# cmavro/GNN-RAG

Hardware: NVIDIA H100
Metric: questions/sec (GNN forward+score) on WebQSP-shape subgraphs; agg-kernel HBM GB/s (higher is better)
Workload: dtype f32

## Files before the change

gnn_rag_b200/csrc/linear_tc.cu:

```cuda
#include "wgmma.cuh"

namespace gr {

int g_tc_cluster = 1;
int g_tc_bk = 32;
int g_tc_tma_store = 1;

namespace {

using namespace tc;
constexpr int kThreads = 384;
constexpr int kConsumerWarps = 8;
constexpr int kLaunchRegs = 168, kProducerRegs = 40, kConsumerRegs = 232;
static_assert(128 * kProducerRegs + 256 * kConsumerRegs <= kThreads * kLaunchRegs, "register budget");

__global__ void split_bf16_seg_kernel(const float* __restrict__ W, int64_t ldw, int64_t N, int64_t Kpad,
                                      int seg, int pitch, __nv_bfloat16* __restrict__ hi,
                                      __nv_bfloat16* __restrict__ lo, int64_t ldo) {
  const int64_t total = N * Kpad;
  const int64_t stride = (int64_t)gridDim.x * blockDim.x;
  for (int64_t i = (int64_t)blockIdx.x * blockDim.x + threadIdx.x; i < total; i += stride) {
    const int64_t n = i / Kpad, k = i - n * Kpad;
    const int sidx = (int)(k / pitch), c = (int)(k - (int64_t)sidx * pitch);
    float v = c < seg ? __ldg(W + n * ldw + (int64_t)sidx * seg + c) : 0.f;
    const __nv_bfloat16 h = __float2bfloat16_rn(v);
    hi[n * ldo + k] = h;
    lo[n * ldo + k] = __float2bfloat16_rn(v - __bfloat162float(h));
  }
}

__global__ void split_bf16_kernel(const float* __restrict__ A, int64_t lda, int64_t M, int64_t K,
                                  __nv_bfloat16* __restrict__ hi, __nv_bfloat16* __restrict__ lo,
                                  int64_t ldo, int vec_ok, int vec_st) {
  const int64_t kq = (K + 3) / 4;
  const int64_t total = M * kq;
  const int64_t stride = (int64_t)gridDim.x * blockDim.x;
  for (int64_t i = (int64_t)blockIdx.x * blockDim.x + threadIdx.x; i < total; i += stride) {
// ... 19 lines not shown
    if (vec_st && k + 3 < ldo) {
      *reinterpret_cast<uint2*>(ph) = *reinterpret_cast<uint2*>(h);
      *reinterpret_cast<uint2*>(pl) = *reinterpret_cast<uint2*>(l);
    } else {
#pragma unroll
      for (int q = 0; q < 4; ++q)
        if (k + q < ldo) { ph[q] = h[q]; pl[q] = l[q]; }
    }
  }
}

struct TcParams {
  const float* bias;
  float* C;
  int64_t ldc;
  __nv_bfloat16* c_hi;
  __nv_bfloat16* c_lo;
  int64_t ldc16;
  const float* w_score;
  float* dots;
  int M, N, K, n_pad, n16, stages, num_tiles;
  uint32_t flags;
  int tma_store;
  int kg_T, kg_G, kg_pitch, kg_nkb, kg_one0, kg_one1, kg_nb0;
};

template <int NP, int CS, int BK, bool GROUPED>
__global__ void __launch_bounds__(kThreads, 1)
linear_tc_kernel(const __grid_constant__ CUtensorMap map_a_hi, const __grid_constant__ CUtensorMap map_a_lo,
                 const __grid_constant__ CUtensorMap map_w_hi, const __grid_constant__ CUtensorMap map_w_lo,
                 const __grid_constant__ CUtensorMap map_c, const __grid_constant__ CUtensorMap map_c_hi,
                 const __grid_constant__ CUtensorMap map_c_lo, const TcParams p) {
  extern __shared__ __align__(1024) uint8_t smem_raw[];
  uint8_t* smem = reinterpret_cast<uint8_t*>((reinterpret_cast<uintptr_t>(smem_raw) + 1023) & ~(uintptr_t)1023);
  const int a_bytes = BM * BK * 2;
  constexpr int w_bytes = NP * BK * 2;
  const bool single = (p.flags & GR_LINEAR_BF16_SINGLE) != 0;
  const int w_off = single ? a_bytes : 2 * a_bytes;
  const int stage_bytes = single ? a_bytes + w_bytes : 2 * a_bytes + 2 * w_bytes;
  uint8_t* s_out = smem + (size_t)p.stages * stage_bytes;
  uint64_t* bars = reinterpret_cast<uint64_t*>(s_out + 2 * kStageOutBytes);
  uint64_t* full_bar = bars;
  uint64_t* empty_bar = bars + p.stages;
  float* s_bias = reinterpret_cast<float*>(bars + 2 * p.stages);
  float* s_ws = s_bias + 256;
  for (int i = threadIdx.x; i < 256; i += kThreads) {
    s_bias[i] = (p.bias && i < p.N) ? p.bias[i] : 0.f;
    s_ws[i] = (p.w_score && i < p.N) ? p.w_score[i] : 0.f;
  }

  const int warp = threadIdx.x >> 5, lane = threadIdx.x & 31;
  const int nkb = GROUPED ? p.kg_nkb : (p.K + BK - 1) / BK;
  const int crank = CS > 1 ? (int)cluster_ctarank() : 0;
  const int ncluster = gridDim.x / CS, cid = blockIdx.x / CS;
  const int ngroups = (p.num_tiles + CS - 1) / CS;
  constexpr uint16_t kMask = (uint16_t)((1u << CS) - 1);

  if (threadIdx.x == 0) {
    for (int s = 0; s < p.stages; ++s) {
      mbar_init(&full_bar[s], 1);
      mbar_init(&empty_bar[s], kConsumerWarps * CS);
    }
    asm volatile("fence.mbarrier_init.release.cluster;" ::: "memory");
  }
  __syncthreads();
  if (CS > 1) cluster_sync_all();

  if (warp < 4) {
    asm volatile("setmaxnreg.dec.sync.aligned.u32 %0;" ::"n"(kProducerRegs));
    if (warp == 0 && lane == 0) {
      uint32_t phase = 0;
      int s = 0;
      constexpr int w_rows = NP / CS;
      const int w_slice = w_rows * BK * 2;
      for (int g = cid; g < ngroups; g += ncluster) {
        const int m0 = (g * CS + crank) * BM;
        for (int kb = 0; kb < nkb; ++kb) {
          mbar_wait(&empty_bar[s], phase ^ 1);
          uint8_t* st = smem + (size_t)s * stage_bytes;
          mbar_expect_tx(&full_bar[s], (uint32_t)stage_bytes);
          int a_col = kb * BK;
          if constexpr (GROUPED) {
            if (p.kg_nb0 == 0) {
              const int g = kb / p.kg_T, t = kb - g * p.kg_T, ni = p.kg_T >> 1;
              const int seg = t == 0 ? 0 : 1 + 2 * ((t - 1) % ni) + (t - 1) / ni;
              a_col = seg * p.kg_pitch + g * BK;
            } else {
              const int g = min(kb / p.kg_T, p.kg_G), t = kb - g * p.kg_T;
              a_col = t == 0 ? g * BK : p.kg_nb0 + (kb - g - 1) * BK;
            }
          }
          tma_load_2d(st, &map_a_hi, &full_bar[s], a_col, m0);
          if (!single) tma_load_2d(st + a_bytes, &map_a_lo, &full_bar[s], a_col, m0);
          if (CS == 1) {
            tma_load_2d(st + w_off, &map_w_hi, &full_bar[s], kb * BK, 0);
            if (!single) tma_load_2d(st + w_off + w_bytes, &map_w_lo, &full_bar[s], kb * BK, 0);
          } else {
            tma_load_2d_mc(st + w_off + crank * w_slice, &map_w_hi, &full_bar[s], kb * BK,
                           crank * w_rows, kMask);
            if (!single)
              tma_load_2d_mc(st + w_off + w_bytes + crank * w_slice, &map_w_lo, &full_bar[s], kb * BK,
                             crank * w_rows, kMask);
          }
          if (++s == p.stages) { s = 0; phase ^= 1; }
        }
      }
    }
  } else {
    asm volatile("setmaxnreg.inc.sync.aligned.u32 %0;" ::"n"(kConsumerRegs));
    const int cw = (warp - 4) >> 2, wq = warp & 3;
    const EpiOut e{s_bias, s_ws, (p.flags & GR_LINEAR_RELU) != 0};
    const int r = wq * 16 + (lane >> 2), cq = lane & 3;
    uint8_t* stg = s_out + (size_t)cw * kStageOutBytes;
    const bool issuer = wq == 0 && lane == 0;
    const bool vec_c = p.C && (p.ldc % 2 == 0) && ((reinterpret_cast<uintptr_t>(p.C) & 7) == 0);
    const bool vec_h = p.c_hi && (p.ldc16 % 2 == 0) && ((reinterpret_cast<uintptr_t>(p.c_hi) & 3) == 0) &&
                       ((reinterpret_cast<uintptr_t>(p.c_lo) & 3) == 0);
    uint32_t phase = 0;
    int s = 0;
    for (int g = cid; g < ngroups; g += ncluster) {
      const int tile = g * CS + crank;
      float acc[NP / 2];
#pragma unroll
      for (int i = 0; i < NP / 2; ++i) acc[i] = 0.f;
      int prev = -1;
      for (int kb = 0; kb < nkb; ++kb) {
        mbar_wait(&full_bar[s], phase);
        const uint32_t sa = smem_u32(smem + (size_t)s * stage_bytes);
        const uint32_t a_row = (uint32_t)(cw * WG_M * BK * 2);
        const uint64_t da_hi = make_smem_desc<BK>(sa + a_row), da_lo = make_smem_desc<BK>(sa + a_bytes + a_row);
        const uint64_t dw_hi = make_smem_desc<BK>(sa + w_off), dw_lo = make_smem_desc<BK>(sa + w_off + w_bytes);
        if constexpr (GROUPED) {
          if (kb >= p.kg_one0 && kb < p.kg_one1) mma_kblock<NP, BK, 1, false>(acc, da_hi, da_lo, dw_hi, dw_lo);
          else mma_kblock<NP, BK, BK / MMA_K, false>(acc, da_hi, da_lo, dw_hi, dw_lo);
        } else if (single) {
          mma_kblock<NP, BK, BK / MMA_K, true>(acc, da_hi, da_lo, dw_hi, dw_lo);
        } else {
          mma_kblock<NP, BK, BK / MMA_K, false>(acc, da_hi, da_lo, dw_hi, dw_lo);
        }
        wgmma_wait<1>();
        if (prev >= 0 && lane == 0) release_slot<CS>(&empty_bar[prev]);
        prev = s;
        if (++s == p.stages) { s = 0; phase ^= 1; }
      }
      wgmma_wait<0>();
      if (prev >= 0 && lane == 0) release_slot<CS>(&empty_bar[prev]);

      const int64_t row0 = (int64_t)tile * BM + cw * WG_M + r;
      float dot0 = 0.f, dot1 = 0.f;
#pragma unroll
      for (int q = 0; q < NP / 16; ++q) {
        const int c0 = 16 * q;
        if (c0 >= p.n_pad) continue;
        float v[8];
        epi_values(acc, q, cq, e, v, dot0, dot1);
        if (p.tma_store) {
          epi_store_tma(v, stg, r, cq, issuer, 1 + cw, &map_c, &map_c_hi, &map_c_lo, p.C != nullptr,
                        p.c_hi != nullptr, c0, tile * BM + cw * WG_M);
          continue;
        }
#pragma unroll
        for (int b = 0; b < 2; ++b) {
          const int col = c0 + 8 * b + 2 * cq;
#pragma unroll
          for (int hr = 0; hr < 2; ++hr) {
            const int64_t row = row0 + 8 * hr;
            if (row >= p.M) continue;
            const float x0 = v[4 * b + 2 * hr], x1 = v[4 * b + 2 * hr + 1];
            if (p.C) {
              float* c = p.C + row * p.ldc + col;
              if (vec_c && col + 1 < p.N) {
                *reinterpret_cast<float2*>(c) = make_float2(x0, x1);
              } else {
                if (col < p.N) c[0] = x0;
                if (col + 1 < p.N) c[1] = x1;
              }
            }
            if (p.c_hi) {
              uint32_t lo;
              const uint32_t hi = split_hi_lo(x0, x1, lo);
              unsigned short* ph = reinterpret_cast<unsigned short*>(p.c_hi + row * p.ldc16 + col);
              unsigned short* pl = reinterpret_cast<unsigned short*>(p.c_lo + row * p.ldc16 + col);
              if (vec_h && col + 1 < p.n16) {
                *reinterpret_cast<uint32_t*>(ph) = hi;
                *reinterpret_cast<uint32_t*>(pl) = lo;
              } else {
                if (col < p.n16) { ph[0] = (unsigned short)(hi & 0xFFFF); pl[0] = (unsigned short)(lo & 0xFFFF); }
                if (col + 1 < p.n16) { ph[1] = (unsigned short)(hi >> 16); pl[1] = (unsigned short)(lo >> 16); }
              }
            }
          }
        }
      }
      epi_dots(dot0, dot1, p.dots, row0, p.M, cq);
    }
    if (p.tma_store && issuer) asm volatile("cp.async.bulk.wait_group 0;" ::: "memory");
  }
  __syncthreads();
  if (CS > 1) cluster_sync_all();
}

struct TcPlan {
  int64_t kp;
  int n_pad, np, stages, bk;
  size_t a_plane_bytes, w_plane_bytes, total_bytes, w_only_bytes, smem_bytes;
  bool ok;
};

TcPlan plan_tc(int64_t M, int64_t N, int64_t K, bool single = false) {
  TcPlan t{};
  const int BK = g_tc_bk == 64 ? 64 : 32;
  t.ok = (N >= 8 && N <= 256 && K >= 8 && M >= 1);
  t.kp = (K + 7) / 8 * 8;
  t.n_pad = (int)((N + 15) / 16 * 16);
  t.np = t.n_pad <= 64 ? 64 : t.n_pad <= 128 ? 128 : t.n_pad <= 208 ? 208 : 256;
  const size_t stage = (single ? 1 : 2) * ((size_t)BM * BK * 2 + (size_t)t.np * BK * 2);
  int stages = (int)((227 * 1024 - 1024 - 2048 - 128 - 2 * kStageOutBytes) / stage);
  t.stages = stages > 8 ? 8 : stages;
  if (t.stages < 2) t.ok = false;
  t.bk = BK;
  t.smem_bytes = (size_t)t.stages * stage + 1024  + 2 * t.stages * 8 + 2 * 256 * 4 + 2 * kStageOutBytes;
  t.a_plane_bytes = align_up((size_t)M * t.kp * 2, 256);
  t.w_plane_bytes = align_up((size_t)N * t.kp * 2, 256);
  t.total_bytes = 2 * t.a_plane_bytes + 2 * t.w_plane_bytes;
  t.w_only_bytes = 2 * t.w_plane_bytes;
  return t;
}


int split_launch(const float* A, int64_t lda, int64_t M, int64_t K, __nv_bfloat16* hi, __nv_bfloat16* lo,
                 int64_t ldo, cudaStream_t stream) {
  int va = (lda % 4 == 0) && ((reinterpret_cast<uintptr_t>(A) & 15) == 0);
  int64_t work = M * ((K + 3) / 4);
  int grid = (int)std::min<int64_t>(ceil_div(work, 256), 32LL * sm_count());
  int vs = (ldo % 4 == 0) && ((reinterpret_cast<uintptr_t>(hi) & 7) == 0) &&
           ((reinterpret_cast<uintptr_t>(lo) & 7) == 0);
  split_bf16_kernel<<<grid, 256, 0, stream>>>(A, lda, M, K, hi, lo, ldo, va, vs);
  GR_CHECK_LAUNCH();
  return GR_OK;
}

template <int NP, int CS, int BK, bool GROUPED = false>
int launch_tc_cs(const CUtensorMap& m_a_hi, const CUtensorMap& m_a_lo, const CUtensorMap& m_w_hi,
                 const CUtensorMap& m_w_lo, const CUtensorMap& m_c, const CUtensorMap& m_c_hi,
                 const CUtensorMap& m_c_lo, const TcPlan& t, const TcParams& p, cudaStream_t stream) {
  const int ngroups = (p.num_tiles + CS - 1) / CS;
  const int nclusters = std::max(1, std::min(ngroups, sm_count() / CS));
  return launch_cluster<linear_tc_kernel<NP, CS, BK, GROUPED>>("gr_linear_tc", kLaunchRegs, CS, nclusters * CS, kThreads,
                                                               t.smem_bytes, stream, m_a_hi, m_a_lo, m_w_hi, m_w_lo,
                                                               m_c, m_c_hi, m_c_lo, p);
}

template <int NP>
int launch_tc_np(const CUtensorMap* const (&m)[7], int cs, const TcPlan& t, const TcParams& p, cudaStream_t stream) {
  if (p.kg_T) {
    if (cs == 2) return launch_tc_cs<NP, 2, 32, true>(*m[0], *m[1], *m[2], *m[3], *m[4], *m[5], *m[6], t, p, stream);
    return launch_tc_cs<NP, 1, 32, true>(*m[0], *m[1], *m[2], *m[3], *m[4], *m[5], *m[6], t, p, stream);
  }
  if (t.bk == 64) {
    if (cs == 2) return launch_tc_cs<NP, 2, 64>(*m[0], *m[1], *m[2], *m[3], *m[4], *m[5], *m[6], t, p, stream);
    return launch_tc_cs<NP, 1, 64>(*m[0], *m[1], *m[2], *m[3], *m[4], *m[5], *m[6], t, p, stream);
  }
  if (cs == 2) return launch_tc_cs<NP, 2, 32>(*m[0], *m[1], *m[2], *m[3], *m[4], *m[5], *m[6], t, p, stream);
  return launch_tc_cs<NP, 1, 32>(*m[0], *m[1], *m[2], *m[3], *m[4], *m[5], *m[6], t, p, stream);
}

int launch_tc(const __nv_bfloat16* a_hi, const __nv_bfloat16* a_lo, int64_t lda16,
              const __nv_bfloat16* w_hi, const __nv_bfloat16* w_lo, int64_t ldw16, const TcPlan& t,
              TcParams p, cudaStream_t stream) {
  p.n_pad = t.n_pad; p.stages = t.stages;
  p.num_tiles = (int)ceil_div(p.M, BM);
  int cs = (g_tc_cluster >= 2 && (t.np / 2) % 8 == 0 && p.num_tiles >= 2) ? 2 : 1;
  CUtensorMap m_a_hi, m_a_lo, m_w_hi, m_w_lo;
  const int64_t w_cols = p.kg_T ? ldw16 : p.K;
  const int64_t a_cols = p.kg_nb0 ? p.kg_nb0 + (int64_t)(p.kg_T - 1) * p.kg_pitch : p.K;
  if (!make_tmap(&m_a_hi, a_hi, p.M, a_cols, lda16, BM, t.bk) || !make_tmap(&m_a_lo, a_lo, p.M, a_cols, lda16, BM, t.bk) ||
      !make_tmap(&m_w_hi, w_hi, p.N, w_cols, ldw16, t.np / cs, t.bk) ||
      !make_tmap(&m_w_lo, w_lo, p.N, w_cols, ldw16, t.np / cs, t.bk)) {
    set_error("gr_linear_tc: cuTensorMapEncodeTiled failed (pointers must be 16-byte aligned, row strides "
              "multiples of 8 elements)");
    return GR_ERR_CUDA;
  }
  p.n16 = (int)std::min<int64_t>((p.N + 15) / 16 * 16, p.ldc16);
  CUtensorMap m_c, m_c_hi, m_c_lo;
  memset(&m_c, 0, sizeof(m_c)); memset(&m_c_hi, 0, sizeof(m_c_hi)); memset(&m_c_lo, 0, sizeof(m_c_lo));
  bool ok = g_tc_tma_store != 0;
  if (ok && p.C) ok = p.N % 4 == 0 && make_out_tmap(&m_c, p.C, p.M, p.N, p.ldc, 4);
  if (ok && p.c_hi) ok = make_out_tmap(&m_c_hi, p.c_hi, p.M, p.n16, p.ldc16, 2) &&
                         make_out_tmap(&m_c_lo, p.c_lo, p.M, p.n16, p.ldc16, 2);
  p.tma_store = ok ? 1 : 0;
  const CUtensorMap* m[7] = {&m_a_hi, &m_a_lo, &m_w_hi, &m_w_lo, &m_c, &m_c_hi, &m_c_lo};
  switch (t.np) {
    case 64: return launch_tc_np<64>(m, cs, t, p, stream);
    case 128: return launch_tc_np<128>(m, cs, t, p, stream);
    case 208: return launch_tc_np<208>(m, cs, t, p, stream);
    default: return launch_tc_np<256>(m, cs, t, p, stream);
  }
}

}

bool linear_tc_supported(int64_t M, int64_t N, int64_t K) {
  return plan_tc(M, N, K).ok && get_encode_fn() != nullptr;
}

}

extern "C" size_t gr_linear_tc_workspace_bytes(int64_t M, int64_t N, int64_t K) {
  if (M <= 0 || N <= 0 || K <= 0) return 0;
  return gr::plan_tc(M, N, K).total_bytes;
}

extern "C" size_t gr_linear_tc_planes_workspace_bytes(int64_t N, int64_t K) {
  if (N <= 0 || K <= 0) return 0;
  return gr::plan_tc(1, N, K).w_only_bytes;
}

extern "C" int gr_split_bf16(const float* A, int64_t lda, int64_t M, int64_t K, void* hi, void* lo,
                             int64_t ld_out, void* stream_) {
  using namespace gr;
  GR_CHECK_ARG(A && hi && lo, "null pointer");
  GR_CHECK_ARG(M > 0 && K > 0 && lda >= K && ld_out >= K && ld_out % 8 == 0, "bad shape / ld_out % 8 != 0");
  return split_launch(A, lda, M, K, reinterpret_cast<__nv_bfloat16*>(hi), reinterpret_cast<__nv_bfloat16*>(lo),
                      ld_out, reinterpret_cast<cudaStream_t>(stream_));
}

extern "C" int gr_linear_tc(const float* A, int64_t lda, const float* W, int64_t ldw, const float* bias,
                            float* C, int64_t ldc, int64_t M, int64_t N, int64_t K, uint32_t flags,
                            void* workspace, size_t workspace_bytes, void* stream_) {
  using namespace gr;
  cudaStream_t stream = reinterpret_cast<cudaStream_t>(stream_);
  GR_CHECK_ARG(A && W && C && workspace, "null pointer");
  GR_CHECK_ARG(M > 0 && N > 0 && K > 0, "M, N, K must be positive");
  GR_CHECK_ARG(lda >= K && ldw >= K && ldc >= N, "leading dimension smaller than row length");
  GR_CHECK_ARG(M < (int64_t)0x7fffffff - BM, "M exceeds int32 range");
  TcPlan t = plan_tc(M, N, K);
  if (!t.ok) {
    set_error("gr_linear_tc: unsupported shape M=%lld N=%lld K=%lld (need 8 <= N <= 256, K >= 8)",
              (long long)M, (long long)N, (long long)K);
    return GR_ERR_UNSUPPORTED;
  }
  if (int rc = check_workspace(__func__, workspace, workspace_bytes, t.total_bytes)) return rc;
  if ((reinterpret_cast<uintptr_t>(workspace) & 255) != 0) {
    set_error("gr_linear_tc: workspace must be 256-byte aligned");
    return GR_ERR_INVALID_ARG;
  }
  char* ws = reinterpret_cast<char*>(workspace);
  __nv_bfloat16* a_hi = reinterpret_cast<__nv_bfloat16*>(ws);
  __nv_bfloat16* a_lo = reinterpret_cast<__nv_bfloat16*>(ws + t.a_plane_bytes);
  __nv_bfloat16* w_hi = reinterpret_cast<__nv_bfloat16*>(ws + 2 * t.a_plane_bytes);
  __nv_bfloat16* w_lo = reinterpret_cast<__nv_bfloat16*>(ws + 2 * t.a_plane_bytes + t.w_plane_bytes);
  int rc = split_launch(A, lda, M, K, a_hi, a_lo, t.kp, stream);
  if (rc != GR_OK) return rc;
  rc = split_launch(W, ldw, N, K, w_hi, w_lo, t.kp, stream);
  if (rc != GR_OK) return rc;
  TcParams p{};
  p.bias = bias; p.C = C; p.ldc = ldc;
  p.M = (int)M; p.N = (int)N; p.K = (int)K; p.flags = flags;
// ... 8 lines not shown
  using namespace gr;
  cudaStream_t stream = reinterpret_cast<cudaStream_t>(stream_);
  GR_CHECK_ARG(A_hi && (A_lo || (flags & GR_LINEAR_BF16_SINGLE)) && W && workspace, "null pointer");
  GR_CHECK_ARG(C || C_hi, "no output requested");
  GR_CHECK_ARG(M > 0 && N > 0 && K > 0, "M, N, K must be positive");
  const bool grouped = (flags & GR_LINEAR_K_GROUPED) != 0;
  const bool korder = (flags & GR_LINEAR_K_ORDER_PLANES) != 0;
  GR_CHECK_ARG(!korder || grouped, "GR_LINEAR_K_ORDER_PLANES modifies GR_LINEAR_K_GROUPED and needs it");
  if (grouped) {
    GR_CHECK_ARG(k_seg > 0 && k_seg_pitch >= k_seg && k_seg_pitch % 16 == 0,
                 "GR_LINEAR_K_GROUPED needs segmented K: k_seg > 0 and k_seg_pitch >= k_seg, a multiple of 16");
    GR_CHECK_ARG(K % k_seg_pitch == 0 && (K / k_seg_pitch) % 2 == 1,
                 "GR_LINEAR_K_GROUPED needs an odd number of segments (2 I + 1)");
    GR_CHECK_ARG(g_tc_bk != 64, "GR_LINEAR_K_GROUPED needs 32-column k-blocks (tc_bk = 32)");
    GR_CHECK_ARG(!(flags & GR_LINEAR_BF16_SINGLE), "GR_LINEAR_K_GROUPED does not combine with GR_LINEAR_BF16_SINGLE");
  }
  const bool segmented = grouped || (k_seg > 0 && k_seg_pitch > k_seg);
  GR_CHECK_ARG(lda16 >= K && lda16 % 8 == 0, "lda16 must be >= K and a multiple of 8");
  GR_CHECK_ARG(!segmented || K % k_seg_pitch == 0, "K must be a multiple of k_seg_pitch");
  GR_CHECK_ARG(ldw >= (segmented ? K / k_seg_pitch * k_seg : K), "ldw smaller than the weight row length");
  GR_CHECK_ARG(!C || ldc >= N, "ldc smaller than N");
  GR_CHECK_ARG(!C_hi || (C_lo && ldc16 >= N), "C_lo missing or ldc16 smaller than N");
  GR_CHECK_ARG(!dots || w_score, "dots requested without w_score");
  GR_CHECK_ARG(M < (int64_t)0x7fffffff - BM, "M exceeds int32 range");
  TcPlan t = plan_tc(M, N, K, (flags & GR_LINEAR_BF16_SINGLE) != 0);
  if (!t.ok) {
    set_error("gr_linear_tc_planes: unsupported shape M=%lld N=%lld K=%lld", (long long)M, (long long)N,
              (long long)K);
    return GR_ERR_UNSUPPORTED;
  }
  const int num_ins = grouped ? (int)(K / k_seg_pitch / 2) : 0;
  const GroupedK gk = grouped ? plan_grouped_k(k_seg_pitch, num_ins, N, korder) : GroupedK{};
  const int64_t nb0 = (k_seg_pitch + 31) / 32 * 32;
  GR_CHECK_ARG(!korder || lda16 >= nb0 + 2 * num_ins * k_seg_pitch,
               "GR_LINEAR_K_ORDER_PLANES: lda16 must cover the neighbour region (round32(k_seg_pitch) + (K - k_seg_pitch) "
               "columns)");
  const size_t w_plane_bytes = grouped ? gk.w_plane_bytes : t.w_plane_bytes;
  if (workspace_bytes < 2 * w_plane_bytes || (reinterpret_cast<uintptr_t>(workspace) & 255) != 0) {
    set_error("gr_linear_tc_planes: workspace too small or not 256-byte aligned");
    return GR_ERR_WORKSPACE;
  }
  char* ws = reinterpret_cast<char*>(workspace);
  __nv_bfloat16* w_hi = reinterpret_cast<__nv_bfloat16*>(ws);
  __nv_bfloat16* w_lo = reinterpret_cast<__nv_bfloat16*>(ws + w_plane_bytes);
  int rc = GR_OK;
  if (flags & GR_LINEAR_W_PRESPLIT) {
  } else if (grouped) {
// ... 31 lines not shown
```

gnn_rag_b200/csrc/wgmma.cuh:

```cuda
#pragma once
#include <cuda.h>
#include <cuda_bf16.h>

#include "common.cuh"

namespace gr {
namespace tc {

constexpr int BM = 128;
constexpr int WG_M = 64;
constexpr int MMA_K = 16;

struct GroupedK {
  int G, ksteps_last, nkb;
  int64_t kp;
  size_t w_plane_bytes;
};
GroupedK plan_grouped_k(int64_t pitch, int I, int64_t N_out, bool packed = false);
int grouped_w_split(const float* W, int64_t ldw, int64_t N_out, int D, int I, const GroupedK& k, __nv_bfloat16* hi,
                    __nv_bfloat16* lo, cudaStream_t stream);

typedef CUresult (*EncodeTiledFn)(CUtensorMap*, CUtensorMapDataType, cuuint32_t, void*, const cuuint64_t*,
                                  const cuuint64_t*, const cuuint32_t*, const cuuint32_t*,
                                  CUtensorMapInterleave, CUtensorMapSwizzle, CUtensorMapL2promotion,
// ... 166 lines not shown
  } else if constexpr (N == 32) {
    GR_WGMMA(32, GR_REGS16, 16, 17, GR_ACC8(0), GR_ACC8(8));
  } else if constexpr (N == 64) {
    GR_WGMMA(64, GR_REGS32, 32, 33, GR_ACC32(0));
  } else if constexpr (N == 128) {
    GR_WGMMA(128, GR_REGS64, 64, 65, GR_ACC32(0), GR_ACC32(32));
  } else if constexpr (N == 208) {
    GR_WGMMA(208, GR_REGS104, 104, 105, GR_ACC32(0), GR_ACC32(32), GR_ACC32(64), GR_ACC8(96));
  } else {
    static_assert(N == 256, "instruction widths: 16, 32, 64, 128, 208, 256");
    GR_WGMMA(256, GR_REGS128, 128, 129, GR_ACC32(0), GR_ACC32(32), GR_ACC32(64), GR_ACC32(96));
  }
}
#undef GR_WGMMA
#undef GR_REGS128
#undef GR_REGS104
#undef GR_REGS64
#undef GR_REGS32
#undef GR_REGS16
#undef GR_REGS8
#undef GR_ACC32
#undef GR_ACC8

template <int NP, int NI, int BK, int C0 = 0>
__device__ __forceinline__ void wgmma_product(float (&acc)[NP / 2], uint64_t a, uint64_t b) {
  constexpr int n = NP - C0 < NI ? NP - C0 : NI;
  wgmma_bf16<n, C0 / 2>(acc, a, b + (uint64_t)((C0 * BK * 2) >> 4));
  if constexpr (C0 + n < NP) wgmma_product<NP, NI, BK, C0 + n>(acc, a, b);
}

template <int NP, int BK, int KSTEPS, bool SINGLE, int NI = NP>
__device__ __forceinline__ void mma_kblock(float (&acc)[NP / 2], uint64_t da_hi, uint64_t da_lo, uint64_t dw_hi,
                                           uint64_t dw_lo) {
  static_assert(KSTEPS >= 1 && KSTEPS <= BK / MMA_K, "k-steps of one k-block");
  acc_fence(acc);
  wgmma_fence();
#pragma unroll
  for (int k = 0; k < KSTEPS; ++k) {
    const uint64_t adv = (uint64_t)((k * MMA_K * 2) >> 4);
    wgmma_product<NP, NI, BK>(acc, da_hi + adv, dw_hi + adv);
    if (!SINGLE) {
      wgmma_product<NP, NI, BK>(acc, da_hi + adv, dw_lo + adv);
      wgmma_product<NP, NI, BK>(acc, da_lo + adv, dw_hi + adv);
    }
  }
  wgmma_commit();
  acc_fence(acc);
}

struct EpiOut {
  const float* bias;
  const float* w_score;
  bool relu;
};

template <int R>
__device__ __forceinline__ void epi_values(const float (&a)[R], int q, int cq, const EpiOut& e, float (&v)[8],
                                           float& dot0, float& dot1) {
#pragma unroll
  for (int b = 0; b < 2; ++b) {
    const int col = 16 * q + 8 * b + 2 * cq;
    const float2 bb = *reinterpret_cast<const float2*>(e.bias + col);
    const float2 ww = *reinterpret_cast<const float2*>(e.w_score + col);
#pragma unroll
    for (int i = 0; i < 4; ++i) {
      float x = a[8 * q + 4 * b + i] + ((i & 1) ? bb.y : bb.x);
      if (e.relu) x = fmaxf(x, 0.f);
      v[4 * b + i] = x;
    }
    dot0 = fmaf(v[4 * b + 0], ww.x, dot0); dot0 = fmaf(v[4 * b + 1], ww.y, dot0);
    dot1 = fmaf(v[4 * b + 2], ww.x, dot1); dot1 = fmaf(v[4 * b + 3], ww.y, dot1);
  }
}

__device__ __forceinline__ uint32_t split_hi_lo(float x0, float x1, uint32_t& lo) {
  const __nv_bfloat162 h2 = __floats2bfloat162_rn(x0, x1);
  const float2 hf = __bfloat1622float2(h2);
  const __nv_bfloat162 l2 = __floats2bfloat162_rn(x0 - hf.x, x1 - hf.y);
  lo = *reinterpret_cast<const uint32_t*>(&l2);
  return *reinterpret_cast<const uint32_t*>(&h2);
}

constexpr int kStageOutBytes = WG_M * 16 * 4 + 2 * WG_M * 16 * 2;
__device__ __forceinline__ void epi_store_tma(const float (&v)[8], uint8_t* stg, int r, int cq, bool issuer,
                                              int bar_id, const CUtensorMap* map_c, const CUtensorMap* map_hi,
                                              const CUtensorMap* map_lo, bool has_c, bool has_planes, int c0, int m0) {
  if (issuer) asm volatile("cp.async.bulk.wait_group.read 0;" ::: "memory");
  named_bar_sync(bar_id, 128);
  float* s_c = reinterpret_cast<float*>(stg);
  uint32_t* s_h = reinterpret_cast<uint32_t*>(stg + WG_M * 16 * 4);
  uint32_t* s_l = reinterpret_cast<uint32_t*>(stg + WG_M * 16 * 4 + WG_M * 16 * 2);
#pragma unroll
  for (int b = 0; b < 2; ++b) {
    const int col = 8 * b + 2 * cq;
#pragma unroll
    for (int hr = 0; hr < 2; ++hr) {
      const int row = r + 8 * hr;
      const float x0 = v[4 * b + 2 * hr], x1 = v[4 * b + 2 * hr + 1];
      if (has_c) *reinterpret_cast<float2*>(s_c + row * 16 + col) = make_float2(x0, x1);
      if (has_planes) {
        uint32_t lo;
        const uint32_t hi = split_hi_lo(x0, x1, lo);
        s_h[row * 8 + col / 2] = hi;
        s_l[row * 8 + col / 2] = lo;
      }
    }
  }
  asm volatile("fence.proxy.async.shared::cta;" ::: "memory");
  named_bar_sync(bar_id, 128);
  if (issuer) {
    if (has_c) tma_store_2d(map_c, stg, c0, m0);
    if (has_planes) {
      tma_store_2d(map_hi, stg + WG_M * 16 * 4, c0, m0);
      tma_store_2d(map_lo, stg + WG_M * 16 * 4 + WG_M * 16 * 2, c0, m0);
    }
    asm volatile("cp.async.bulk.commit_group;" ::: "memory");
  }
}

__device__ __forceinline__ void epi_dots(float dot0, float dot1, float* dots, int64_t row0, int64_t M, int cq) {
  dot0 += __shfl_xor_sync(0xffffffffu, dot0, 1);
  dot0 += __shfl_xor_sync(0xffffffffu, dot0, 2);
  dot1 += __shfl_xor_sync(0xffffffffu, dot1, 1);
  dot1 += __shfl_xor_sync(0xffffffffu, dot1, 2);
  if (dots && cq == 0) {
    if (row0 < M) { dots[row0] = dot0; dots[M + row0] = 0.f; }
    if (row0 + 8 < M) { dots[row0 + 8] = dot1; dots[M + row0 + 8] = 0.f; }
  }
}

template <auto Kernel, typename... Args>
int launch_cluster(const char* fn, int launch_regs, int cs, int grid, int threads, size_t smem, cudaStream_t stream,
                   const Args&... args) {
  if (int rc = opt_in_smem<Kernel>(fn, 227 * 1024)) return rc;
  static int num_regs = 0;
  if (num_regs == 0) {
    cudaFuncAttributes fa{};
// ... 27 lines not shown
```

include/gnnrag_b200.h:

```cpp
#ifndef GNNRAG_B200_H_
#define GNNRAG_B200_H_

#include <stddef.h>
#include <stdint.h>

#ifdef __cplusplus
extern "C" {
#endif

#define GR_ABI_VERSION 1

typedef enum gr_status {
  GR_OK = 0,
  GR_ERR_INVALID_ARG = -1,
  GR_ERR_CUDA = -2,
  GR_ERR_WORKSPACE = -3,
  GR_ERR_UNSUPPORTED = -4
} gr_status;

#define GR_LINEAR_RELU 1u
#define GR_LINEAR_EXACT_FP32 2u
#define GR_LINEAR_BF16_SINGLE 8u
#define GR_LINEAR_W_PRESPLIT 4u

// ... 3 lines not shown
int gr_abi_version(void);
const char* gr_last_error(void);
int gr_set_option(const char* name, int64_t value);
static inline int64_t gr_pad4(int64_t n) { return (n + 3) & ~(int64_t)3; }

size_t gr_csr_build_workspace_bytes(int64_t F, int64_t Nt);
int gr_csr_build(const void* heads, const void* rels, const void* tails, int idx_bytes,
                 int64_t F, int64_t Nt, int64_t num_rel_rows,
                 int32_t* rowptr_t, int32_t* src_t, int32_t* rel_t, int32_t* fact_t,
                 int32_t* rowptr_h, int32_t* src_h, int32_t* rel_h, int32_t* fact_h,
                 int32_t* status, const int32_t* nfacts, void* workspace, size_t workspace_bytes, void* stream);

int gr_gather_f32(const float* in, const int32_t* fact, float* out, int64_t F, void* stream);

int gr_linear(const float* A, int64_t lda, const float* W, int64_t ldw, const float* bias,
              const float* addend, int64_t ld_addend, int64_t addend_rows,
              float* C, int64_t ldc, int64_t M, int64_t N, int64_t K, uint32_t flags, void* stream);

size_t gr_linear_tc_workspace_bytes(int64_t M, int64_t N, int64_t K);
int gr_linear_tc(const float* A, int64_t lda, const float* W, int64_t ldw, const float* bias,
                 float* C, int64_t ldc, int64_t M, int64_t N, int64_t K, uint32_t flags,
                 void* workspace, size_t workspace_bytes, void* stream);
size_t gr_linear_tc_planes_workspace_bytes(int64_t N, int64_t K);
int gr_linear_tc_planes(const void* A_hi, const void* A_lo, int64_t lda16, const float* W, int64_t ldw,
                        const float* bias, float* C, int64_t ldc, void* C_hi, void* C_lo, int64_t ldc16,
                        const float* w_score, float* dots, int64_t M, int64_t N, int64_t K,
                        int64_t k_seg, int64_t k_seg_pitch,
                        uint32_t flags, void* workspace, size_t workspace_bytes, void* stream);
int gr_split_bf16(const float* A, int64_t lda, int64_t M, int64_t K, void* hi, void* lo, int64_t ld_out,
                  void* stream);

int gr_aggregate(const int32_t* rowptr, const int32_t* src, const int32_t* rel, const float* w,
                 const float* prior, const float* table, const float* ins,
                 float* out, int64_t out_row_stride, int64_t out_col0, int64_t seg_stride,
                 float* possible, int B, int N, int D, int I, int64_t F, void* stream);

int gr_aggregate_backward(const int32_t* rowptr, const int32_t* src, const int32_t* rel, const float* w,
                          const float* prior, const float* table, const float* ins, const float* grad_out,
                          int64_t grad_row_stride, int64_t grad_col0, int64_t seg_stride, float* grad_table,
                          float* grad_ins, float* grad_prior, int B, int N, int D, int I, int64_t F, void* stream);

int gr_aggregate_dual(const int32_t* rowptr_t, const int32_t* src_t, const int32_t* rel_t,
                      const float* w_t, const int32_t* rowptr_h, const int32_t* src_h,
                      const int32_t* rel_h, const float* w_h, const float* prior,
                      const float* table_fwd, const float* table_inv, const float* ins,
                      float* out, int64_t out_row_stride, int64_t out_col0, int64_t seg_pitch,
// ... 292 lines not shown
```

Measured before the change: 12920.

## Add 256-row M tiles for single-plane BF16 tensor-core linear

```diff
diff --git a/gnn_rag_b200/csrc/linear_tc.cu b/gnn_rag_b200/csrc/linear_tc.cu
--- a/gnn_rag_b200/csrc/linear_tc.cu
+++ b/gnn_rag_b200/csrc/linear_tc.cu
@@ -11,8 +11,12 @@
 using namespace tc;
 constexpr int kThreads = 384;
 constexpr int kConsumerWarps = 8;
-constexpr int kLaunchRegs = 168, kProducerRegs = 40, kConsumerRegs = 232;
-static_assert(128 * kProducerRegs + 256 * kConsumerRegs <= kThreads * kLaunchRegs, "register budget");
+constexpr int kLaunchRegs = 168;
+template <int TM> constexpr int kProducerRegs = TM == 256 ? 24 : 40;
+template <int TM> constexpr int kConsumerRegs = TM == 256 ? 240 : 232;
+static_assert(128 * kProducerRegs<128> + 256 * kConsumerRegs<128> <= kThreads * kLaunchRegs, "register budget");
+static_assert(128 * kProducerRegs<256> + 256 * kConsumerRegs<256> <= kThreads * kLaunchRegs, "register budget");
+constexpr int kTileRowsWide = 256, kWideMaxNP = 208;
 
 __global__ void split_bf16_seg_kernel(const float* __restrict__ W, int64_t ldw, int64_t N, int64_t Kpad,
                                       int seg, int pitch, __nv_bfloat16* __restrict__ hi,
@@ -78,24 +82,28 @@
   int M, N, K, n_pad, n16, stages, num_tiles;
   uint32_t flags;
   int tma_store;
+  int out_stage;
   int kg_T, kg_G, kg_pitch, kg_nkb, kg_one0, kg_one1, kg_nb0;
 };
 
-template <int NP, int CS, int BK, bool GROUPED>
+template <int NP, int CS, int BK, bool GROUPED, int TM>
 __global__ void __launch_bounds__(kThreads, 1)
 linear_tc_kernel(const __grid_constant__ CUtensorMap map_a_hi, const __grid_constant__ CUtensorMap map_a_lo,
                  const __grid_constant__ CUtensorMap map_w_hi, const __grid_constant__ CUtensorMap map_w_lo,
                  const __grid_constant__ CUtensorMap map_c, const __grid_constant__ CUtensorMap map_c_hi,
                  const __grid_constant__ CUtensorMap map_c_lo, const TcParams p) {
   extern __shared__ __align__(1024) uint8_t smem_raw[];
-  uint8_t* smem = reinterpret_cast<uint8_t*>((reinterpret_cast<uintptr_t>(smem_raw) + 1023) & ~(uintptr_t)1023);
-  const int a_bytes = BM * BK * 2;
+  uint8_t* smem = smem_raw + ((1024u - (smem_u32(smem_raw) & 1023u)) & 1023u);
+  static_assert(TM == BM || (TM == kTileRowsWide && NP <= kWideMaxNP && CS == 1 && !GROUPED), "tile rows");
+  constexpr int MH = TM / BM;
+  constexpr int RW = TM / 2;
+  const int a_bytes = TM * BK * 2;
   constexpr int w_bytes = NP * BK * 2;
-  const bool single = (p.flags & GR_LINEAR_BF16_SINGLE) != 0;
+  const bool single = TM == kTileRowsWide || (p.flags & GR_LINEAR_BF16_SINGLE) != 0;
   const int w_off = single ? a_bytes : 2 * a_bytes;
   const int stage_bytes = single ? a_bytes + w_bytes : 2 * a_bytes + 2 * w_bytes;
   uint8_t* s_out = smem + (size_t)p.stages * stage_bytes;
-  uint64_t* bars = reinterpret_cast<uint64_t*>(s_out + 2 * kStageOutBytes);
+  uint64_t* bars = reinterpret_cast<uint64_t*>(s_out + 2 * p.out_stage);
   uint64_t* full_bar = bars;
   uint64_t* empty_bar = bars + p.stages;
   float* s_bias = reinterpret_cast<float*>(bars + 2 * p.stages);
@@ -123,14 +131,14 @@
   if (CS > 1) cluster_sync_all();
 
   if (warp < 4) {
-    asm volatile("setmaxnreg.dec.sync.aligned.u32 %0;" ::"n"(kProducerRegs));
+    asm volatile("setmaxnreg.dec.sync.aligned.u32 %0;" ::"n"(kProducerRegs<TM>));
     if (warp == 0 && lane == 0) {
       uint32_t phase = 0;
       int s = 0;
       constexpr int w_rows = NP / CS;
       const int w_slice = w_rows * BK * 2;
       for (int g = cid; g < ngroups; g += ncluster) {
-        const int m0 = (g * CS + crank) * BM;
+        const int m0 = (g * CS + crank) * TM;
         for (int kb = 0; kb < nkb; ++kb) {
           mbar_wait(&empty_bar[s], phase ^ 1);
           uint8_t* st = smem + (size_t)s * stage_bytes;
@@ -163,36 +171,30 @@
       }
     }
   } else {
-    asm volatile("setmaxnreg.inc.sync.aligned.u32 %0;" ::"n"(kConsumerRegs));
+    asm volatile("setmaxnreg.inc.sync.aligned.u32 %0;" ::"n"(kConsumerRegs<TM>));
     const int cw = (warp - 4) >> 2, wq = warp & 3;
-    const EpiOut e{s_bias, s_ws, (p.flags & GR_LINEAR_RELU) != 0};
-    const int r = wq * 16 + (lane >> 2), cq = lane & 3;
-    uint8_t* stg = s_out + (size_t)cw * kStageOutBytes;
     const bool issuer = wq == 0 && lane == 0;
-    const bool vec_c = p.C && (p.ldc % 2 == 0) && ((reinterpret_cast<uintptr_t>(p.C) & 7) == 0);
-    const bool vec_h = p.c_hi && (p.ldc16 % 2 == 0) && ((reinterpret_cast<uintptr_t>(p.c_hi) & 3) == 0) &&
-                       ((reinterpret_cast<uintptr_t>(p.c_lo) & 3) == 0);
     uint32_t phase = 0;
     int s = 0;
     for (int g = cid; g < ngroups; g += ncluster) {
       const int tile = g * CS + crank;
-      float acc[NP / 2];
-#pragma unroll
-      for (int i = 0; i < NP / 2; ++i) acc[i] = 0.f;
+      float acc[MH * NP / 2];
+#pragma unroll
+      for (int i = 0; i < MH * NP / 2; ++i) acc[i] = 0.f;
       int prev = -1;
       for (int kb = 0; kb < nkb; ++kb) {
         mbar_wait(&full_bar[s], phase);
         const uint32_t sa = smem_u32(smem + (size_t)s * stage_bytes);
-        const uint32_t a_row = (uint32_t)(cw * WG_M * BK * 2);
+        const uint32_t a_row = (uint32_t)(cw * RW * BK * 2);
         const uint64_t da_hi = make_smem_desc<BK>(sa + a_row), da_lo = make_smem_desc<BK>(sa + a_bytes + a_row);
         const uint64_t dw_hi = make_smem_desc<BK>(sa + w_off), dw_lo = make_smem_desc<BK>(sa + w_off + w_bytes);
         if constexpr (GROUPED) {
-          if (kb >= p.kg_one0 && kb < p.kg_one1) mma_kblock<NP, BK, 1, false>(acc, da_hi, da_lo, dw_hi, dw_lo);
-          else mma_kblock<NP, BK, BK / MMA_K, false>(acc, da_hi, da_lo, dw_hi, dw_lo);
+          if (kb >= p.kg_one0 && kb < p.kg_one1) mma_kblock<NP, BK, 1, false, NP, MH>(acc, da_hi, da_lo, dw_hi, dw_lo);
+          else mma_kblock<NP, BK, BK / MMA_K, false, NP, MH>(acc, da_hi, da_lo, dw_hi, dw_lo);
         } else if (single) {
-          mma_kblock<NP, BK, BK / MMA_K, true>(acc, da_hi, da_lo, dw_hi, dw_lo);
+          mma_kblock<NP, BK, BK / MMA_K, true, NP, MH>(acc, da_hi, da_lo, dw_hi, dw_lo);
         } else {
-          mma_kblock<NP, BK, BK / MMA_K, false>(acc, da_hi, da_lo, dw_hi, dw_lo);
+          mma_kblock<NP, BK, BK / MMA_K, false, NP, MH>(acc, da_hi, da_lo, dw_hi, dw_lo);
         }
         wgmma_wait<1>();
         if (prev >= 0 && lane == 0) release_slot<CS>(&empty_bar[prev]);
@@ -202,53 +204,67 @@
       wgmma_wait<0>();
       if (prev >= 0 && lane == 0) release_slot<CS>(&empty_bar[prev]);
 
-      const int64_t row0 = (int64_t)tile * BM + cw * WG_M + r;
-      float dot0 = 0.f, dot1 = 0.f;
-#pragma unroll
-      for (int q = 0; q < NP / 16; ++q) {
-        const int c0 = 16 * q;
-        if (c0 >= p.n_pad) continue;
-        float v[8];
-        epi_values(acc, q, cq, e, v, dot0, dot1);
-        if (p.tma_store) {
-          epi_store_tma(v, stg, r, cq, issuer, 1 + cw, &map_c, &map_c_hi, &map_c_lo, p.C != nullptr,
-                        p.c_hi != nullptr, c0, tile * BM + cw * WG_M);
-          continue;
-        }
-#pragma unroll
-        for (int b = 0; b < 2; ++b) {
-          const int col = c0 + 8 * b + 2 * cq;
-#pragma unroll
-          for (int hr = 0; hr < 2; ++hr) {
-            const int64_t row = row0 + 8 * hr;
-            if (row >= p.M) continue;
-            const float x0 = v[4 * b + 2 * hr], x1 = v[4 * b + 2 * hr + 1];
-            if (p.C) {
-              float* c = p.C + row * p.ldc + col;
-              if (vec_c && col + 1 < p.N) {
-                *reinterpret_cast<float2*>(c) = make_float2(x0, x1);
-              } else {
-                if (col < p.N) c[0] = x0;
-                if (col + 1 < p.N) c[1] = x1;
-              }
-            }
-            if (p.c_hi) {
-              uint32_t lo;
-              const uint32_t hi = split_hi_lo(x0, x1, lo);
-              unsigned short* ph = reinterpret_cast<unsigned short*>(p.c_hi + row * p.ldc16 + col);
-              unsigned short* pl = reinterpret_cast<unsigned short*>(p.c_lo + row * p.ldc16 + col);
-              if (vec_h && col + 1 < p.n16) {
-                *reinterpret_cast<uint32_t*>(ph) = hi;
-                *reinterpret_cast<uint32_t*>(pl) = lo;
-              } else {
-                if (col < p.n16) { ph[0] = (unsigned short)(hi & 0xFFFF); pl[0] = (unsigned short)(lo & 0xFFFF); }
-                if (col + 1 < p.n16) { ph[1] = (unsigned short)(hi >> 16); pl[1] = (unsigned short)(lo >> 16); }
+      const auto epilogue = [&](auto h) {
+        constexpr int H = decltype(h)::value;
+        const EpiOut e{s_bias, s_ws, (p.flags & GR_LINEAR_RELU) != 0};
+        const int r = wq * 16 + (lane >> 2), cq = lane & 3;
+        uint8_t* stg = s_out + (size_t)cw * p.out_stage;
+        const int m0 = tile * TM + cw * RW + WG_M * H;
+        const int64_t row0 = (int64_t)m0 + r;
+        float dot0 = 0.f, dot1 = 0.f;
+#pragma unroll
+        for (int q = 0; q < NP / 16; ++q) {
+          const int c0 = 16 * q;
+          if (c0 >= p.n_pad) continue;
+          float v[8];
+          epi_values<H * NP / 2>(acc, q, cq, e, v, dot0, dot1);
+          if (p.tma_store || TM == kTileRowsWide) {
+            epi_store_tma(v, stg, r, cq, issuer, 1 + cw, &map_c, &map_c_hi, &map_c_lo, p.C != nullptr,
+                          p.c_hi != nullptr, c0, m0);
+            continue;
+          }
+          if constexpr (TM == BM) {
+            const bool vec_c = p.C && (p.ldc % 2 == 0) && ((reinterpret_cast<uintptr_t>(p.C) & 7) == 0);
+            const bool vec_h = p.c_hi && (p.ldc16 % 2 == 0) && ((reinterpret_cast<uintptr_t>(p.c_hi) & 3) == 0) &&
+                               ((reinterpret_cast<uintptr_t>(p.c_lo) & 3) == 0);
+#pragma unroll
+            for (int b = 0; b < 2; ++b) {
+              const int col = c0 + 8 * b + 2 * cq;
+#pragma unroll
+              for (int hr = 0; hr < 2; ++hr) {
+                const int64_t row = row0 + 8 * hr;
+                if (row >= p.M) continue;
+                const float x0 = v[4 * b + 2 * hr], x1 = v[4 * b + 2 * hr + 1];
+                if (p.C) {
+                  float* c = p.C + row * p.ldc + col;
+                  if (vec_c && col + 1 < p.N) {
+                    *reinterpret_cast<float2*>(c) = make_float2(x0, x1);
+                  } else {
+                    if (col < p.N) c[0] = x0;
+                    if (col + 1 < p.N) c[1] = x1;
+                  }
+                }
+                if (p.c_hi) {
+                  uint32_t lo;
+                  const uint32_t hi = split_hi_lo(x0, x1, lo);
+                  unsigned short* ph = reinterpret_cast<unsigned short*>(p.c_hi + row * p.ldc16 + col);
+                  unsigned short* pl = reinterpret_cast<unsigned short*>(p.c_lo + row * p.ldc16 + col);
+                  if (vec_h && col + 1 < p.n16) {
+                    *reinterpret_cast<uint32_t*>(ph) = hi;
+                    *reinterpret_cast<uint32_t*>(pl) = lo;
+                  } else {
+                    if (col < p.n16) { ph[0] = (unsigned short)(hi & 0xFFFF); pl[0] = (unsigned short)(lo & 0xFFFF); }
+                    if (col + 1 < p.n16) { ph[1] = (unsigned short)(hi >> 16); pl[1] = (unsigned short)(lo >> 16); }
+                  }
+                }
               }
             }
           }
         }
-      }
-      epi_dots(dot0, dot1, p.dots, row0, p.M, cq);
+        epi_dots(dot0, dot1, p.dots, row0, p.M, cq);
+      };
+      epilogue(std::integral_constant<int, 0>{});
+      if constexpr (MH == 2) epilogue(std::integral_constant<int, 1>{});
     }
     if (p.tma_store && issuer) asm volatile("cp.async.bulk.wait_group 0;" ::: "memory");
   }
@@ -259,23 +275,34 @@
 struct TcPlan {
   int64_t kp;
   int n_pad, np, stages, bk;
+  int tm;
   size_t a_plane_bytes, w_plane_bytes, total_bytes, w_only_bytes, smem_bytes;
   bool ok;
 };
 
-TcPlan plan_tc(int64_t M, int64_t N, int64_t K, bool single = false) {
+int np_of(int n_pad) { return n_pad <= 64 ? 64 : n_pad <= 128 ? 128 : n_pad <= 208 ? 208 : 256; }
+
+int tc_tile_rows(int64_t M, int64_t N, uint32_t flags, int sms) {
+  const int np = np_of((int)((N + 15) / 16 * 16));
+  const bool wide = (flags & GR_LINEAR_BF16_SINGLE) && !(flags & GR_LINEAR_K_GROUPED) && np <= kWideMaxNP &&
+                    g_tc_bk != 64 && g_tc_cluster < 2 && ceil_div(M, (int64_t)kTileRowsWide) >= sms;
+  return wide ? kTileRowsWide : BM;
+}
+
+TcPlan plan_tc(int64_t M, int64_t N, int64_t K, bool single = false, int tm = BM, int out_stage = kStageOutBytes) {
   TcPlan t{};
   const int BK = g_tc_bk == 64 ? 64 : 32;
   t.ok = (N >= 8 && N <= 256 && K >= 8 && M >= 1);
   t.kp = (K + 7) / 8 * 8;
   t.n_pad = (int)((N + 15) / 16 * 16);
-  t.np = t.n_pad <= 64 ? 64 : t.n_pad <= 128 ? 128 : t.n_pad <= 208 ? 208 : 256;
-  const size_t stage = (single ? 1 : 2) * ((size_t)BM * BK * 2 + (size_t)t.np * BK * 2);
-  int stages = (int)((227 * 1024 - 1024 - 2048 - 128 - 2 * kStageOutBytes) / stage);
+  t.np = np_of(t.n_pad);
+  t.tm = tm;
+  const size_t stage = (single ? 1 : 2) * ((size_t)tm * BK * 2 + (size_t)t.np * BK * 2);
+  int stages = (int)((227 * 1024 - 1024 - 2048 - 128 - 2 * out_stage) / stage);
   t.stages = stages > 8 ? 8 : stages;
   if (t.stages < 2) t.ok = false;
   t.bk = BK;
-  t.smem_bytes = (size_t)t.stages * stage + 1024  + 2 * t.stages * 8 + 2 * 256 * 4 + 2 * kStageOutBytes;
+  t.smem_bytes = (size_t)t.stages * stage + 1024  + 2 * t.stages * 8 + 2 * 256 * 4 + 2 * out_stage;
   t.a_plane_bytes = align_up((size_t)M * t.kp * 2, 256);
   t.w_plane_bytes = align_up((size_t)N * t.kp * 2, 256);
   t.total_bytes = 2 * t.a_plane_bytes + 2 * t.w_plane_bytes;
@@ -296,19 +323,24 @@
   return GR_OK;
 }
 
-template <int NP, int CS, int BK, bool GROUPED = false>
+template <int NP, int CS, int BK, bool GROUPED = false, int TM = BM>
 int launch_tc_cs(const CUtensorMap& m_a_hi, const CUtensorMap& m_a_lo, const CUtensorMap& m_w_hi,
                  const CUtensorMap& m_w_lo, const CUtensorMap& m_c, const CUtensorMap& m_c_hi,
                  const CUtensorMap& m_c_lo, const TcPlan& t, const TcParams& p, cudaStream_t stream) {
   const int ngroups = (p.num_tiles + CS - 1) / CS;
   const int nclusters = std::max(1, std::min(ngroups, sm_count() / CS));
-  return launch_cluster<linear_tc_kernel<NP, CS, BK, GROUPED>>("gr_linear_tc", kLaunchRegs, CS, nclusters * CS, kThreads,
-                                                               t.smem_bytes, stream, m_a_hi, m_a_lo, m_w_hi, m_w_lo,
-                                                               m_c, m_c_hi, m_c_lo, p);
+  return launch_cluster<linear_tc_kernel<NP, CS, BK, GROUPED, TM>>("gr_linear_tc", kLaunchRegs, CS, nclusters * CS,
+                                                                   kThreads, t.smem_bytes, stream, m_a_hi, m_a_lo,
+                                                                   m_w_hi, m_w_lo, m_c, m_c_hi, m_c_lo, p);
 }
 
 template <int NP>
 int launch_tc_np(const CUtensorMap* const (&m)[7], int cs, const TcPlan& t, const TcParams& p, cudaStream_t stream) {
+  if constexpr (NP <= kWideMaxNP) {
+    if (t.tm == kTileRowsWide)
+      return launch_tc_cs<NP, 1, 32, false, kTileRowsWide>(*m[0], *m[1], *m[2], *m[3], *m[4], *m[5], *m[6], t, p,
+                                                           stream);
+  }
   if (p.kg_T) {
     if (cs == 2) return launch_tc_cs<NP, 2, 32, true>(*m[0], *m[1], *m[2], *m[3], *m[4], *m[5], *m[6], t, p, stream);
     return launch_tc_cs<NP, 1, 32, true>(*m[0], *m[1], *m[2], *m[3], *m[4], *m[5], *m[6], t, p, stream);
@@ -322,21 +354,8 @@
 }
 
 int launch_tc(const __nv_bfloat16* a_hi, const __nv_bfloat16* a_lo, int64_t lda16,
-              const __nv_bfloat16* w_hi, const __nv_bfloat16* w_lo, int64_t ldw16, const TcPlan& t,
+              const __nv_bfloat16* w_hi, const __nv_bfloat16* w_lo, int64_t ldw16, TcPlan t,
               TcParams p, cudaStream_t stream) {
-  p.n_pad = t.n_pad; p.stages = t.stages;
-  p.num_tiles = (int)ceil_div(p.M, BM);
-  int cs = (g_tc_cluster >= 2 && (t.np / 2) % 8 == 0 && p.num_tiles >= 2) ? 2 : 1;
-  CUtensorMap m_a_hi, m_a_lo, m_w_hi, m_w_lo;
-  const int64_t w_cols = p.kg_T ? ldw16 : p.K;
-  const int64_t a_cols = p.kg_nb0 ? p.kg_nb0 + (int64_t)(p.kg_T - 1) * p.kg_pitch : p.K;
-  if (!make_tmap(&m_a_hi, a_hi, p.M, a_cols, lda16, BM, t.bk) || !make_tmap(&m_a_lo, a_lo, p.M, a_cols, lda16, BM, t.bk) ||
-      !make_tmap(&m_w_hi, w_hi, p.N, w_cols, ldw16, t.np / cs, t.bk) ||
-      !make_tmap(&m_w_lo, w_lo, p.N, w_cols, ldw16, t.np / cs, t.bk)) {
-    set_error("gr_linear_tc: cuTensorMapEncodeTiled failed (pointers must be 16-byte aligned, row strides "
-              "multiples of 8 elements)");
-    return GR_ERR_CUDA;
-  }
   p.n16 = (int)std::min<int64_t>((p.N + 15) / 16 * 16, p.ldc16);
   CUtensorMap m_c, m_c_hi, m_c_lo;
   memset(&m_c, 0, sizeof(m_c)); memset(&m_c_hi, 0, sizeof(m_c_hi)); memset(&m_c_lo, 0, sizeof(m_c_lo));
@@ -345,6 +364,23 @@
   if (ok && p.c_hi) ok = make_out_tmap(&m_c_hi, p.c_hi, p.M, p.n16, p.ldc16, 2) &&
                          make_out_tmap(&m_c_lo, p.c_lo, p.M, p.n16, p.ldc16, 2);
   p.tma_store = ok ? 1 : 0;
+  p.out_stage = p.tma_store && !p.C ? kStagePlaneBytes : kStageOutBytes;
+  const int tm = p.tma_store && tc_tile_rows(p.M, p.N, p.flags, sm_count()) == kTileRowsWide ? kTileRowsWide : BM;
+  t = plan_tc(p.M, p.N, p.K, (p.flags & GR_LINEAR_BF16_SINGLE) != 0, tm, p.out_stage);
+  p.n_pad = t.n_pad; p.stages = t.stages;
+  p.num_tiles = (int)ceil_div(p.M, t.tm);
+  const int cs = (t.tm == BM && g_tc_cluster >= 2 && (t.np / 2) % 8 == 0 && p.num_tiles >= 2) ? 2 : 1;
+  CUtensorMap m_a_hi, m_a_lo, m_w_hi, m_w_lo;
+  const int64_t w_cols = p.kg_T ? ldw16 : p.K;
+  const int64_t a_cols = p.kg_nb0 ? p.kg_nb0 + (int64_t)(p.kg_T - 1) * p.kg_pitch : p.K;
+  if (!make_tmap(&m_a_hi, a_hi, p.M, a_cols, lda16, t.tm, t.bk) ||
+      !make_tmap(&m_a_lo, a_lo, p.M, a_cols, lda16, t.tm, t.bk) ||
+      !make_tmap(&m_w_hi, w_hi, p.N, w_cols, ldw16, t.np / cs, t.bk) ||
+      !make_tmap(&m_w_lo, w_lo, p.N, w_cols, ldw16, t.np / cs, t.bk)) {
+    set_error("gr_linear_tc: cuTensorMapEncodeTiled failed (pointers must be 16-byte aligned, row strides "
+              "multiples of 8 elements)");
+    return GR_ERR_CUDA;
+  }
   const CUtensorMap* m[7] = {&m_a_hi, &m_a_lo, &m_w_hi, &m_w_lo, &m_c, &m_c_hi, &m_c_lo};
   switch (t.np) {
     case 64: return launch_tc_np<64>(m, cs, t, p, stream);
@@ -360,6 +396,11 @@
   return plan_tc(M, N, K).ok && get_encode_fn() != nullptr;
 }
 
+}
+
+extern "C" int gr_linear_tc_tile_rows(int64_t M, int64_t N, uint32_t flags, int sms) {
+  if (M <= 0 || N <= 0 || N > 256) return 0;
+  return gr::tc_tile_rows(M, N, flags, sms > 0 ? sms : gr::sm_count());
 }
 
 extern "C" size_t gr_linear_tc_workspace_bytes(int64_t M, int64_t N, int64_t K) {
@@ -389,7 +430,7 @@
   GR_CHECK_ARG(A && W && C && workspace, "null pointer");
   GR_CHECK_ARG(M > 0 && N > 0 && K > 0, "M, N, K must be positive");
   GR_CHECK_ARG(lda >= K && ldw >= K && ldc >= N, "leading dimension smaller than row length");
-  GR_CHECK_ARG(M < (int64_t)0x7fffffff - BM, "M exceeds int32 range");
+  GR_CHECK_ARG(M < (int64_t)0x7fffffff - kTileRowsWide, "M exceeds int32 range");
   TcPlan t = plan_tc(M, N, K);
   if (!t.ok) {
     set_error("gr_linear_tc: unsupported shape M=%lld N=%lld K=%lld (need 8 <= N <= 256, K >= 8)",
@@ -444,7 +485,7 @@
   GR_CHECK_ARG(!C || ldc >= N, "ldc smaller than N");
   GR_CHECK_ARG(!C_hi || (C_lo && ldc16 >= N), "C_lo missing or ldc16 smaller than N");
   GR_CHECK_ARG(!dots || w_score, "dots requested without w_score");
-  GR_CHECK_ARG(M < (int64_t)0x7fffffff - BM, "M exceeds int32 range");
+  GR_CHECK_ARG(M < (int64_t)0x7fffffff - kTileRowsWide, "M exceeds int32 range");
   TcPlan t = plan_tc(M, N, K, (flags & GR_LINEAR_BF16_SINGLE) != 0);
   if (!t.ok) {
     set_error("gr_linear_tc_planes: unsupported shape M=%lld N=%lld K=%lld", (long long)M, (long long)N,
diff --git a/gnn_rag_b200/csrc/wgmma.cuh b/gnn_rag_b200/csrc/wgmma.cuh
--- a/gnn_rag_b200/csrc/wgmma.cuh
+++ b/gnn_rag_b200/csrc/wgmma.cuh
@@ -212,15 +212,22 @@
 #undef GR_ACC32
 #undef GR_ACC8
 
-template <int NP, int NI, int BK, int C0 = 0>
-__device__ __forceinline__ void wgmma_product(float (&acc)[NP / 2], uint64_t a, uint64_t b) {
+template <int NP, int NI, int BK, int C0 = 0, int OFF = 0, int R>
+__device__ __forceinline__ void wgmma_product(float (&acc)[R], uint64_t a, uint64_t b) {
   constexpr int n = NP - C0 < NI ? NP - C0 : NI;
-  wgmma_bf16<n, C0 / 2>(acc, a, b + (uint64_t)((C0 * BK * 2) >> 4));
-  if constexpr (C0 + n < NP) wgmma_product<NP, NI, BK, C0 + n>(acc, a, b);
-}
-
-template <int NP, int BK, int KSTEPS, bool SINGLE, int NI = NP>
-__device__ __forceinline__ void mma_kblock(float (&acc)[NP / 2], uint64_t da_hi, uint64_t da_lo, uint64_t dw_hi,
+  wgmma_bf16<n, OFF + C0 / 2>(acc, a, b + (uint64_t)((C0 * BK * 2) >> 4));
+  if constexpr (C0 + n < NP) wgmma_product<NP, NI, BK, C0 + n, OFF>(acc, a, b);
+}
+
+template <int NP, int NI, int BK, int MH>
+__device__ __forceinline__ void wgmma_rows(float (&acc)[MH * NP / 2], uint64_t a, uint64_t b) {
+  static_assert(MH == 1 || MH == 2, "one or two 64-row blocks per warpgroup");
+  wgmma_product<NP, NI, BK>(acc, a, b);
+  if constexpr (MH == 2) wgmma_product<NP, NI, BK, 0, NP / 2>(acc, a + (uint64_t)((WG_M * BK * 2) >> 4), b);
+}
+
+template <int NP, int BK, int KSTEPS, bool SINGLE, int NI = NP, int MH = 1>
+__device__ __forceinline__ void mma_kblock(float (&acc)[MH * NP / 2], uint64_t da_hi, uint64_t da_lo, uint64_t dw_hi,
                                            uint64_t dw_lo) {
   static_assert(KSTEPS >= 1 && KSTEPS <= BK / MMA_K, "k-steps of one k-block");
   acc_fence(acc);
@@ -228,10 +235,10 @@
 #pragma unroll
   for (int k = 0; k < KSTEPS; ++k) {
     const uint64_t adv = (uint64_t)((k * MMA_K * 2) >> 4);
-    wgmma_product<NP, NI, BK>(acc, da_hi + adv, dw_hi + adv);
+    wgmma_rows<NP, NI, BK, MH>(acc, da_hi + adv, dw_hi + adv);
     if (!SINGLE) {
-      wgmma_product<NP, NI, BK>(acc, da_hi + adv, dw_lo + adv);
-      wgmma_product<NP, NI, BK>(acc, da_lo + adv, dw_hi + adv);
+      wgmma_rows<NP, NI, BK, MH>(acc, da_hi + adv, dw_lo + adv);
+      wgmma_rows<NP, NI, BK, MH>(acc, da_lo + adv, dw_hi + adv);
     }
   }
   wgmma_commit();
@@ -244,7 +251,7 @@
   bool relu;
 };
 
-template <int R>
+template <int OFF = 0, int R>
 __device__ __forceinline__ void epi_values(const float (&a)[R], int q, int cq, const EpiOut& e, float (&v)[8],
                                            float& dot0, float& dot1) {
 #pragma unroll
@@ -254,7 +261,7 @@
     const float2 ww = *reinterpret_cast<const float2*>(e.w_score + col);
 #pragma unroll
     for (int i = 0; i < 4; ++i) {
-      float x = a[8 * q + 4 * b + i] + ((i & 1) ? bb.y : bb.x);
+      float x = a[OFF + 8 * q + 4 * b + i] + ((i & 1) ? bb.y : bb.x);
       if (e.relu) x = fmaxf(x, 0.f);
       v[4 * b + i] = x;
     }
@@ -272,14 +279,16 @@
 }
 
 constexpr int kStageOutBytes = WG_M * 16 * 4 + 2 * WG_M * 16 * 2;
+constexpr int kStagePlaneBytes = 2 * WG_M * 16 * 2;
 __device__ __forceinline__ void epi_store_tma(const float (&v)[8], uint8_t* stg, int r, int cq, bool issuer,
                                               int bar_id, const CUtensorMap* map_c, const CUtensorMap* map_hi,
                                               const CUtensorMap* map_lo, bool has_c, bool has_planes, int c0, int m0) {
   if (issuer) asm volatile("cp.async.bulk.wait_group.read 0;" ::: "memory");
   named_bar_sync(bar_id, 128);
   float* s_c = reinterpret_cast<float*>(stg);
-  uint32_t* s_h = reinterpret_cast<uint32_t*>(stg + WG_M * 16 * 4);
-  uint32_t* s_l = reinterpret_cast<uint32_t*>(stg + WG_M * 16 * 4 + WG_M * 16 * 2);
+  const int pl = has_c ? WG_M * 16 * 4 : 0;
+  uint32_t* s_h = reinterpret_cast<uint32_t*>(stg + pl);
+  uint32_t* s_l = reinterpret_cast<uint32_t*>(stg + pl + WG_M * 16 * 2);
 #pragma unroll
   for (int b = 0; b < 2; ++b) {
     const int col = 8 * b + 2 * cq;
@@ -301,8 +310,8 @@
   if (issuer) {
     if (has_c) tma_store_2d(map_c, stg, c0, m0);
     if (has_planes) {
-      tma_store_2d(map_hi, stg + WG_M * 16 * 4, c0, m0);
-      tma_store_2d(map_lo, stg + WG_M * 16 * 4 + WG_M * 16 * 2, c0, m0);
+      tma_store_2d(map_hi, stg + pl, c0, m0);
+      tma_store_2d(map_lo, stg + pl + WG_M * 16 * 2, c0, m0);
     }
     asm volatile("cp.async.bulk.commit_group;" ::: "memory");
   }
diff --git a/include/gnnrag_b200.h b/include/gnnrag_b200.h
--- a/include/gnnrag_b200.h
+++ b/include/gnnrag_b200.h
@@ -49,6 +49,7 @@
                  float* C, int64_t ldc, int64_t M, int64_t N, int64_t K, uint32_t flags,
                  void* workspace, size_t workspace_bytes, void* stream);
 size_t gr_linear_tc_planes_workspace_bytes(int64_t N, int64_t K);
+int gr_linear_tc_tile_rows(int64_t M, int64_t N, uint32_t flags, int sms);
 int gr_linear_tc_planes(const void* A_hi, const void* A_lo, int64_t lda16, const float* W, int64_t ldw,
                         const float* bias, float* C, int64_t ldc, void* C_hi, void* C_lo, int64_t ldc16,
                         const float* w_score, float* dots, int64_t M, int64_t N, int64_t K,
```

New measurement: 13260 (median of 6 runs). 2.6% higher.
